# fanshiqing/mpiT

Measured on AMD Instinct MI355X. Metric: images/sec (whole node) ResNet-50 async-SGD at 1/2/4/8 MI355X, higher is better.
Workload: dtype fp32; 1 GPU; model=resnet50, global_batch=256, image_size=224, parallelism=async-ps-colocated-1srv-1wrk, optimizer=downpour, su=1, per_gpu_batch=256, master_weights=fp32, defer_ps_wait=False

## Files before the change

csrc/bindings.cpp:

```cpp
#include <pybind11/pybind11.h>
#include <pybind11/stl.h>

#include "core/engine.h"
#include "core/ps.h"
#include "core/window.h"
#include "kernels/kernels.h"
#include "kernels/stem_pack.h"

namespace py = pybind11;
using namespace mpit;

namespace {
hipStream_t S(uintptr_t s) { return reinterpret_cast<hipStream_t>(s); }
py::tuple st_tuple(const Status& s) { return py::make_tuple(s.source, s.tag, s.error, s.count, s.cancelled); }
}

static void apply_sfold(BnRed& r, const py::object& f) {
  if (f.is_none()) return;
  auto t = f.cast<py::tuple>();
  if (t.size() != 11 && t.size() != 12) throw std::invalid_argument("bn fold: 11 or 12 fields");
  r.scoef = t[0].cast<uintptr_t>();
  r.sgamma = t[1].cast<uintptr_t>();
  r.sbeta = t[2].cast<uintptr_t>();
  r.srmean = t[3].cast<uintptr_t>();
// ... 176 lines not shown
      py::arg("oepoch") = 0);
  m.def("gemm_nt_fold_lvl_floats", &gemm_nt_fold_lvl_floats);
  m.def("bound_floats", [] { return kBoundFloats; });
  m.def("gemm_tn_supported", &gemm_tn_supported);
  m.def("gemm_tn_ws_floats", &gemm_tn_ws_floats);
  m.def("device_cu_count", &device_cu_count);
  m.def("stream_create_cu_masked", &stream_create_cu_masked);
  m.def(
      "gemm_tn",
      [](int dev, uintptr_t s, int64_t M, int N, int K, uintptr_t Y, int64_t ldy, uintptr_t X, int64_t ldx,
         uintptr_t out, uintptr_t ws, float beta, bool f32, uintptr_t amax_y, uintptr_t amax_x, int64_t yps,
         int64_t xps) {
        gemm_tn(dev, S(s), M, N, K, Y, ldy, X, ldx, out, ws, beta, f32, amax_y, amax_x, yps, xps);
      },
      py::arg("dev"), py::arg("stream"), py::arg("M"), py::arg("N"), py::arg("K"), py::arg("Y"), py::arg("ldy"),
      py::arg("X"), py::arg("ldx"), py::arg("out"), py::arg("ws"), py::arg("beta"), py::arg("f32") = false,
      py::arg("amax_y") = 0, py::arg("amax_x") = 0, py::arg("yps") = 0, py::arg("xps") = 0);
  m.def(
      "cast_transpose",
      [](int dev, uintptr_t s, uintptr_t w, int R, int Cc, uintptr_t wb, uintptr_t wt, int taps, bool f32) {
        cast_transpose(dev, S(s), w, R, Cc, wb, wt, taps, f32);
      },
      py::arg("dev"), py::arg("stream"), py::arg("w"), py::arg("R"), py::arg("Cc"), py::arg("wb"), py::arg("wt"),
      py::arg("taps") = 1, py::arg("f32") = false);
  m.def("cast_job_bytes", &cast_job_bytes);
  m.def("cast_jobs_build", [](uintptr_t table, std::vector<std::array<int64_t, 11>> specs) {
    return cast_jobs_build(table, specs);
  });
  m.def(
      "cast_jobs_run",
      [](int dev, uintptr_t s, uintptr_t table, int njobs, int64_t nblocks, uintptr_t amax) {
        cast_jobs_run(dev, S(s), table, njobs, nblocks, amax);
      },
      py::arg("dev"), py::arg("s"), py::arg("table"), py::arg("njobs"), py::arg("nblocks"), py::arg("amax") = 0);
  m.def(
      "maxpool_fwd",
      [](int dev, uintptr_t s, int N, int H, int W, int C, int K, int stride, int pad, uintptr_t x, uintptr_t y,
         uintptr_t idx, bool f32, uintptr_t ibound, uintptr_t obound) {
        maxpool_fwd(dev, S(s), N, H, W, C, K, stride, pad, x, y, idx, f32, ibound, obound);
      },
      py::arg("dev"), py::arg("stream"), py::arg("N"), py::arg("H"), py::arg("W"), py::arg("C"), py::arg("K"),
      py::arg("stride"), py::arg("pad"), py::arg("x"), py::arg("y"), py::arg("idx"), py::arg("f32") = false,
      py::arg("ibound") = 0, py::arg("obound") = 0);
  m.def(
      "maxpool_bwd",
      [](int dev, uintptr_t s, int N, int H, int W, int C, int K, int stride, int pad, uintptr_t dy, uintptr_t idx,
         uintptr_t dx, bool f32, uintptr_t ypool, uintptr_t db, uintptr_t ws) {
        maxpool_bwd(dev, S(s), N, H, W, C, K, stride, pad, dy, idx, dx, f32, ypool, db, ws);
      },
      py::arg("dev"), py::arg("stream"), py::arg("N"), py::arg("H"), py::arg("W"), py::arg("C"), py::arg("K"),
      py::arg("stride"), py::arg("pad"), py::arg("dy"), py::arg("idx"), py::arg("dx"), py::arg("f32") = false,
      py::arg("ypool") = 0, py::arg("db") = 0, py::arg("ws") = 0);
  m.def("maxpool_bwd_ws_floats", &maxpool_bwd_ws_floats);
  m.def(
      "avgpool_bwd",
      [](int dev, uintptr_t s, int N, int HW, int C, uintptr_t dy, uintptr_t dx, bool f32) {
        avgpool_bwd(dev, S(s), N, HW, C, dy, dx, f32);
      },
      py::arg("dev"), py::arg("stream"), py::arg("N"), py::arg("HW"), py::arg("C"), py::arg("dy"), py::arg("dx"),
      py::arg("f32") = false);
  m.def("col_sums_ws_floats", &col_sums_ws_floats);
  m.def(
      "col_sums",
      [](int dev, uintptr_t s, uintptr_t part, int64_t nb, int64_t ld, int C, uintptr_t out, uintptr_t mid) {
        col_sums(dev, S(s), part, nb, ld, C, out, mid);
      },
      py::arg("dev"), py::arg("stream"), py::arg("part"), py::arg("nb"), py::arg("ld"), py::arg("C"), py::arg("out"),
      py::arg("mid") = 0);
  m.def("conv_supported", &conv_supported);
  m.def(
      "conv_fwd",
      [](int dev, uintptr_t s, int Nb, int H, int W, int C, int Co, int R, int S_, int stride, int pad, uintptr_t x,
         uintptr_t w, uintptr_t y, uintptr_t stats, uintptr_t cin, uintptr_t bias, bool relu, uintptr_t red_part,
         uintptr_t red_x, uintptr_t red_mask, uintptr_t red_mean, int64_t red_row0, uintptr_t red_part2,
         uintptr_t red_x2, uintptr_t red_mean2, bool f32, uintptr_t fold_coef, uintptr_t fold_gamma,
         uintptr_t fold_rstd, uintptr_t fold_dgamma, uintptr_t fold_dbeta, uintptr_t fold_lvl, int64_t bps,
         uintptr_t amax_a, uintptr_t amax_b, uintptr_t fold_zero, py::object bn_fold, bool red_relu,
         bool fold_tag, int64_t aps, uintptr_t omax, uint32_t oepoch) {
        BnRed r{red_part, red_x, red_mask, red_mean, red_row0, red_part2, red_x2, red_mean2};
        r.fcoef = fold_coef; r.fgamma = fold_gamma; r.frstd = fold_rstd;
        r.fdgamma = fold_dgamma; r.fdbeta = fold_dbeta; r.flvl = fold_lvl; r.fzero = fold_zero;
        r.amax_a = amax_a; r.amax_b = amax_b; r.aps = aps; r.omax = omax; r.oepoch = oepoch;
        r.relu_y = red_relu ? 1 : 0;
        r.ftag = fold_tag ? 1 : 0;
        apply_sfold(r, bn_fold);
        conv_fwd(dev, S(s), Nb, H, W, C, Co, R, S_, stride, pad, x, w, y, stats, cin, bias, relu, &r, f32, bps);
      },
      py::arg("dev"), py::arg("stream"), py::arg("Nb"), py::arg("H"), py::arg("W"), py::arg("C"), py::arg("Co"),
      py::arg("R"), py::arg("S"), py::arg("stride"), py::arg("pad"), py::arg("x"), py::arg("w"), py::arg("y"),
      py::arg("stats") = 0, py::arg("cin") = 0, py::arg("bias") = 0, py::arg("relu") = false, py::arg("red_part") = 0,
      py::arg("red_x") = 0, py::arg("red_mask") = 0, py::arg("red_mean") = 0, py::arg("red_row0") = 0,
      py::arg("red_part2") = 0, py::arg("red_x2") = 0, py::arg("red_mean2") = 0, py::arg("f32") = false,
      py::arg("fold_coef") = 0, py::arg("fold_gamma") = 0, py::arg("fold_rstd") = 0, py::arg("fold_dgamma") = 0,
      py::arg("fold_dbeta") = 0, py::arg("fold_lvl") = 0, py::arg("bps") = 0, py::arg("amax_a") = 0,
      py::arg("amax_b") = 0, py::arg("fold_zero") = 0, py::arg("bn_fold") = py::none(), py::arg("red_relu") = false,
      py::arg("fold_tag") = false, py::arg("aps") = 0, py::arg("omax") = 0, py::arg("oepoch") = 0);
  m.def("conv_dgrad_strided_wfloats", &conv_dgrad_strided_wfloats);
  m.def(
      "conv_dgrad_strided_weights",
      [](int dev, uintptr_t s, uintptr_t w, int Co, int C, int R, int S_, int stride, int pad, uintptr_t wb,
         uintptr_t wcls, bool f32) { conv_dgrad_strided_weights(dev, S(s), w, Co, C, R, S_, stride, pad, wb, wcls, f32); },
      py::arg("dev"), py::arg("stream"), py::arg("w"), py::arg("Co"), py::arg("C"), py::arg("R"), py::arg("S"),
      py::arg("stride"), py::arg("pad"), py::arg("wb"), py::arg("wcls"), py::arg("f32") = false);
  m.def("conv_dgrad_strided_tiles", &conv_dgrad_strided_tiles);
  m.def(
      "conv_dgrad_strided",
// ... 358 lines not shown
```

csrc/kernels/bn_act.hip:

```cpp
#include <hip/hip_runtime.h>

#include <atomic>
#include <cmath>
#include <stdexcept>
#include <cstdlib>
#include <string>
#include <type_traits>

#include "ew.h"
#include "kernels.h"
#include "planes.h"

namespace mpit {
namespace {

constexpr int kMaxStatBlocks = 512;
constexpr int kFinCh = 64;
constexpr int kFinK = 16;

template <typename T>
struct Vec;
template <>
struct Vec<uint16_t> {
  static constexpr int N = 8;
// ... 934 lines not shown
  check_shape(M, C, V, reinterpret_cast<uintptr_t>(x));
  if (relu && !mask) throw std::invalid_argument("bn_act backward: ReLU needs the forward mask");
  const int G = C / V;
  const int blk = block_for(G);
  const int R = blk / G;
  int64_t rpb;
  const int nb = stat_blocks(M, R, &rpb);
  const float* coef = coef_in ? coef_in : ws;
  float* part = ws + 3 * C;
  const size_t shm = size_t(R) * 2 * C * sizeof(float);
  if (coef_in) {
  } else if (gpart) {
    FinArgs fa{};
    fa.gamma = gamma;
    fa.mean = mean;
    fa.rstd = rstd;
    fa.dgamma = dgamma;
    fa.dbeta = dbeta;
    fa.coef = ws;
    fa.zero = reinterpret_cast<float*>(amax);
    launch_tiles_finalize<T, false>(s, gpart, npart, C, M, x, part, fa);
  } else {
    if (relu)
      hipLaunchKernelGGL((bn_bwd_reduce_kernel<T, true>), dim3(nb), dim3(blk), shm, s, dy, mask, x, mean, M, C, rpb,
                         part);
    else
      hipLaunchKernelGGL((bn_bwd_reduce_kernel<T, false>), dim3(nb), dim3(blk), shm, s, dy, mask, x, mean, M, C, rpb,
                         part);
    hipLaunchKernelGGL(bn_finalize_bwd_kernel, dim3((C + kFinCh - 1) / kFinCh), dim3(kFinCh * kFinK), 0, s, part, nb,
                       C, M, gamma, mean, rstd, dgamma, dbeta, ws);
    if (amax) hip_check(hipMemsetAsync(reinterpret_cast<void*>(amax), 0, kBoundFloats * sizeof(float), s), "amax zero");
  }
  const int64_t nvec = M * G;
  const int u = apply_u(sizeof(T) == 4);
  const dim3 g(apply_grid_u(nvec, blk, u)), b(blk);
  if (!dx) {
    hip_check(hipGetLastError(), "bn_act backward launch");
    return;
  }
  with_mode<sizeof(T) == 4>(split_ok(sizeof(T) == 4, C, blk), u, [&](auto sp, auto uu) {
    constexpr bool SP = decltype(sp)::value;
    constexpr int U = decltype(uu)::value;
    if (relu) {
      if (dres) hipLaunchKernelGGL((bn_bwd_apply_kernel<T, true, true, SP, U>), g, b, 0, s, dy, mask, x, coef, dx, dres, nvec, C, am);
      else hipLaunchKernelGGL((bn_bwd_apply_kernel<T, true, false, SP, U>), g, b, 0, s, dy, mask, x, coef, dx, dres, nvec, C, am);
    } else {
      if (dres) hipLaunchKernelGGL((bn_bwd_apply_kernel<T, false, true, SP, U>), g, b, 0, s, dy, mask, x, coef, dx, dres, nvec, C, am);
      else hipLaunchKernelGGL((bn_bwd_apply_kernel<T, false, false, SP, U>), g, b, 0, s, dy, mask, x, coef, dx, dres, nvec, C, am);
    }
  });
  hip_check(hipGetLastError(), "bn_act backward launch");
}

}

int64_t bn_workspace_floats(int C) { return int64_t(3) * C + int64_t(2) * kMaxStatBlocks * C; }

int64_t bn_mask_bytes(bool bf16, int64_t M, int C) { (void)bf16; return M * (C / 8); }

void bn_act_fwd(int dev, hipStream_t s, bool bf16, uintptr_t x, uintptr_t res, uintptr_t y, int64_t M, int C,
                uintptr_t gamma, uintptr_t beta, uintptr_t rmean, uintptr_t rvar, uintptr_t save_mean,
                uintptr_t save_rstd, uintptr_t ws, float momentum, float eps, bool relu, uintptr_t mask,
                uintptr_t stats, int64_t nstat, uintptr_t amax, uintptr_t coef, const PlaneSpec* planes) {
  hip_check(hipSetDevice(dev), "hipSetDevice");
  if (planes && (bf16 || (planes->obound && !y) || (planes->rplanes && !(res && planes->rbound)) ||
                 (planes->obound && res && !planes->rbound)))
    throw std::invalid_argument("bn_act forward: fp16 planes are for fp32 passes with the bounds of their inputs");
  auto F = [](uintptr_t p) { return reinterpret_cast<float*>(p); };
  auto* mk = reinterpret_cast<uint8_t*>(mask);
  if (coef) {
    if (!y) throw std::invalid_argument("bn_act forward: given coefficients need y");
    if (bf16) {
      check_shape(M, C, 8, x);
      launch_apply<uint16_t>(s, reinterpret_cast<const uint16_t*>(x), reinterpret_cast<const uint16_t*>(res),
                             reinterpret_cast<uint16_t*>(y), M, C, F(coef), relu, mk, AmaxOut{F(amax)});
    } else {
      check_shape(M, C, 8, x);
      launch_apply<float>(s, reinterpret_cast<const float*>(x), reinterpret_cast<const float*>(res),
                          reinterpret_cast<float*>(y), M, C, F(coef), relu, mk, amax_out(amax, planes));
    }
    hip_check(hipGetLastError(), "bn_act forward launch");
    return;
  }
  if (bf16)
    fwd_impl<uint16_t>(dev, s, reinterpret_cast<const uint16_t*>(x), reinterpret_cast<const uint16_t*>(res),
                       reinterpret_cast<uint16_t*>(y), M, C, F(gamma), F(beta), F(rmean), F(rvar), F(save_mean),
                       F(save_rstd), F(ws), momentum, eps, relu, mk, F(stats), nstat, amax, nullptr);
  else
    fwd_impl<float>(dev, s, reinterpret_cast<const float*>(x), reinterpret_cast<const float*>(res),
                    reinterpret_cast<float*>(y), M, C, F(gamma), F(beta), F(rmean), F(rvar), F(save_mean), F(save_rstd),
                    F(ws), momentum, eps, relu, mk, F(stats), nstat, amax, planes);
}

void bn_act_apply(int dev, hipStream_t s, bool bf16, uintptr_t x, uintptr_t res, uintptr_t y, int64_t M, int C,
                  uintptr_t coef, bool relu) {
  hip_check(hipSetDevice(dev), "hipSetDevice");
  if (bf16) {
    check_shape(M, C, 8, x);
    launch_apply<uint16_t>(s, reinterpret_cast<const uint16_t*>(x), reinterpret_cast<const uint16_t*>(res),
                           reinterpret_cast<uint16_t*>(y), M, C, reinterpret_cast<const float*>(coef), relu, nullptr);
  } else {
    check_shape(M, C, 8, x);
    launch_apply<float>(s, reinterpret_cast<const float*>(x), reinterpret_cast<const float*>(res),
                        reinterpret_cast<float*>(y), M, C, reinterpret_cast<const float*>(coef), relu, nullptr);
  }
  hip_check(hipGetLastError(), "bn_act apply launch");
// ... 81 lines not shown
```

csrc/kernels/kernels.h:

```cpp
#pragma once
#include <hip/hip_runtime.h>
#include <cstdint>
#include <array>
#include <vector>

namespace mpit {

enum Rule : int {
  kApply = 0,
  kApplySum = 1,
  kRMSProp = 2,
  kAdam = 3,
  kAdamax = 4,
  kAdagrad = 5,
  kAdadelta = 6,
  kNesterovPre = 7,
  kNesterovPost = 8,
  kDownpour = 9,
  kElastic = 10,
  kRegClip = 11,
  kScale = 12,
  kCopy = 13,
  kFill = 14,
  kAxpby = 15,
// ... 108 lines not shown
                        uintptr_t dy, uintptr_t wcls, uintptr_t dx, const BnRed* red = nullptr, bool f32 = false,
                        int64_t bps = 0);
void softmax_xent(int dev, hipStream_t s, int64_t rows, int C, uintptr_t x, int64_t ldx, bool bf16, uintptr_t tgt,
                  float scale, uintptr_t loss, uintptr_t d);

void seq_hidden_windows(int dev, hipStream_t s, uintptr_t tok, int64_t B, int T, uintptr_t E, int D, uintptr_t Wh,
                        uintptr_t bh, int H, int k, uintptr_t out, int Kp);
void seq_max_norm(int dev, hipStream_t s, uintptr_t c, int64_t ldc, uintptr_t tok, int64_t B, int T, int k,
                  int64_t pad_idx, uintptr_t bias, int F, float eps, uintptr_t out);
void gesd_gather(int dev, hipStream_t s, uintptr_t q, uintptr_t cand, uintptr_t idx, int64_t n, int w, int D,
                 uintptr_t out);

void seq_max_norm_arg(int dev, hipStream_t s, uintptr_t c, int64_t ldc, uintptr_t tok, int64_t B, int T, int k,
                      int64_t pad_idx, uintptr_t bias, int F, float eps, uintptr_t out, uintptr_t arg, uintptr_t den);
void gesd_pair_bwd(int dev, hipStream_t s, uintptr_t y, int64_t n, int F, float margin, uintptr_t err, uintptr_t sc,
                   uintptr_t gy);
void seq_norm_max_bwd(int dev, hipStream_t s, uintptr_t gy, uintptr_t y, uintptr_t arg, uintptr_t den, int64_t S, int T,
                      int F, int Fp, float eps, uintptr_t dm, uintptr_t dc);
void seq_conv_wgrad_pe(int dev, hipStream_t s, uintptr_t dm, uintptr_t arg, uintptr_t win, int64_t n, int T, int F,
                       int H, int k, int Kp, uintptr_t g, int64_t ldg, int64_t offW, int64_t offB);
void seq_hidden_bwd(int dev, hipStream_t s, uintptr_t dwin, int64_t ldw, uintptr_t win, int Kp, int64_t S, int T, int H,
                    int k, uintptr_t Wh, int D, uintptr_t da, uintptr_t de);
void seq_hidden_embed_grad_pe(int dev, hipStream_t s, uintptr_t da, uintptr_t de, uintptr_t tok, uintptr_t E,
                              int64_t V, int64_t n, int T, int H, int D, int64_t pad_idx, uintptr_t g, int64_t ldg,
                              int64_t offE, int64_t offWh, int64_t offBh);
int64_t relu_bias_bwd_ws_floats(int C);
int64_t col_sums_ws_floats(int C);
void col_sums(hipStream_t s, const float* part, int64_t nb, int64_t ld, int C, float* out, float* mid);
void col_sums(int dev, hipStream_t s, uintptr_t part, int64_t nb, int64_t ld, int C, uintptr_t out, uintptr_t mid);
void relu_bias_bwd(int dev, hipStream_t s, int64_t M, int C, uintptr_t dy, uintptr_t y, uintptr_t dz, uintptr_t db,
                   uintptr_t ws, bool f32 = false);
int64_t conv_wgrad_ws_floats(int dev, int Nb, int H, int W, int C, int Co, int R, int S, int stride, int pad);
void conv_wgrad(int dev, hipStream_t s, int Nb, int H, int W, int C, int Co, int R, int S, int stride, int pad,
                uintptr_t dy, uintptr_t x, uintptr_t dw, uintptr_t ws, float beta, bool f32 = false,
                uintptr_t amax_y = 0, uintptr_t amax_x = 0, int64_t yps = 0,
                int64_t xps = 0);

void conv_stem_fwd(int dev, hipStream_t s, int Nb, int Hp, int Wp, int Co, int Ho, int Wo, int stride, uintptr_t x,
                   uintptr_t w, uintptr_t y, uintptr_t stats, bool f32 = false, int64_t bps = 0, uintptr_t amax_a = 0,
                   uintptr_t amax_b = 0, const BnRed* fold = nullptr, int rows = 8, uintptr_t bias = 0,
                   bool relu = false);
int64_t conv_stem_wgrad_ws_floats(int dev, int Nb, int Ho, int Wo, int Co, int rows = 8);
void conv_stem_wgrad(int dev, hipStream_t s, int Nb, int Hp, int Wp, int Co, int Ho, int Wo, int stride, uintptr_t dy,
                     uintptr_t x, uintptr_t dw, uintptr_t ws, bool f32 = false, uintptr_t amax_y = 0,
                     uintptr_t amax_x = 0, int rows = 8);
int stem_wgrad_rows(int rows);

void maxpool_fwd(int dev, hipStream_t s, int N, int H, int W, int C, int K, int stride, int pad, uintptr_t x,
                 uintptr_t y, uintptr_t idx, bool f32 = false, uintptr_t ibound = 0, uintptr_t obound = 0);
void maxpool_bwd(int dev, hipStream_t s, int N, int H, int W, int C, int K, int stride, int pad, uintptr_t dy,
                 uintptr_t idx, uintptr_t dx, bool f32 = false, uintptr_t ypool = 0, uintptr_t db = 0,
                 uintptr_t ws = 0);
int64_t maxpool_bwd_ws_floats(int C);
void avgpool_bwd(int dev, hipStream_t s, int N, int HW, int C, uintptr_t dy, uintptr_t dx, bool f32 = false);

enum PeerOp : int { kPrSum = 0, kPrProd, kPrMax, kPrMin, kPrLand, kPrLor, kPrLxor, kPrBand, kPrBor, kPrBxor, kPrOps };
enum PeerDtype : int { kPrF32 = 0, kPrBf16, kPrF16, kPrF64, kPrI32, kPrI64, kPrU8, kPrDtypes };
constexpr int kPeerMax = 8;
bool peer_reduce_supported(int op, int dtype);
int peer_dtype_size(int dtype);
void peer_reduce(int dev, hipStream_t s, int op, int dtype, const std::vector<uintptr_t>& srcs,
                 const std::vector<uintptr_t>& dsts, int64_t n);

void type_copy(int dev, hipStream_t s, int dir, uintptr_t strided, uintptr_t packed,
               const std::vector<std::array<int64_t, 2>>& loops, uintptr_t table, int64_t R, int64_t L, int64_t per,
               int unit, int max_blocks = 0, bool wide = false);

}
```

mpit_amd/models/resnet.py:

```python
from __future__ import annotations

from typing import List, Type, Union

import os

import torch
import torch.nn as nn

from ..ops.bn import BatchNormAct2d, bn_pair
from ..ops.conv import Conv1x1, ConvNHWC, GradSlot, StemConv, feeds_bn, park_grad
from ..ops.linear import LinearAct
from ..ops.pool import GlobalAvgPoolNHWC, MaxPool2dNHWC

FUSED_BN = True


def _bn(c, act):
    return BatchNormAct2d(c, act=act) if FUSED_BN else nn.BatchNorm2d(c)


def _feeds_bn(*pairs):
    for p in pairs:
        if p is None:
            continue
        if isinstance(p, nn.Sequential):
            if not (len(p) == 2 and isinstance(p[1], BatchNormAct2d)):
                continue
            p = (p[0], p[1])
        c, bn = p
        if FUSED_BN and hasattr(c, "emit_stats") and isinstance(bn, BatchNormAct2d):
            feeds_bn(c, bn)


MFMA_CONV = os.environ.get("MPIT_MFMA_CONV", "1") != "0"
MFMA_CONV3 = MFMA_CONV and os.environ.get("MPIT_MFMA_CONV3", "1") != "0"
_FC_FP32 = os.environ.get("MPIT_FC_FP32", "0") != "0"


def conv3x3(i, o, stride=1):
    if MFMA_CONV3:
        return ConvNHWC(i, o, 3, stride=stride, padding=1)
    return nn.Conv2d(i, o, 3, stride=stride, padding=1, bias=False)


def conv1x1(i, o, stride=1):
    if MFMA_CONV:
        return Conv1x1(i, o) if stride == 1 else ConvNHWC(i, o, 1, stride=stride)
    return nn.Conv2d(i, o, 1, stride=stride, bias=False)


class BasicBlock(nn.Module):
    expansion = 1

    def __init__(self, inp, planes, stride=1, downsample=None):
        super().__init__()
        self.conv1 = conv3x3(inp, planes, stride)
        self.bn1 = _bn(planes, True)
        self.relu = nn.ReLU(inplace=True)
        self.conv2 = conv3x3(planes, planes)
        self.bn2 = _bn(planes, True)
        self.downsample = downsample
        _feeds_bn((self.conv1, self.bn1), (self.conv2, self.bn2), downsample)
# ... 64 lines not shown
        self.relu = nn.ReLU(inplace=True)
        self.maxpool = MaxPool2dNHWC(3, stride=2, padding=1) if MFMA_CONV else nn.MaxPool2d(3, stride=2, padding=1)
        self.layer1 = self._make(block, 64, layers[0])
        self.layer2 = self._make(block, 128, layers[1], 2)
        self.layer3 = self._make(block, 256, layers[2], 2)
        self.layer4 = self._make(block, 512, layers[3], 2)
        self.avgpool = GlobalAvgPoolNHWC() if MFMA_CONV else nn.AdaptiveAvgPool2d(1)
        self.fc = (LinearAct(512 * block.expansion, num_classes, act=False, pad_out=True) if MFMA_CONV
                   else nn.Linear(512 * block.expansion, num_classes))
        for m in self.modules():
            if isinstance(m, nn.Conv2d):
                nn.init.kaiming_normal_(m.weight, mode="fan_out", nonlinearity="relu")
            elif isinstance(m, nn.BatchNorm2d):
                nn.init.ones_(m.weight)
                nn.init.zeros_(m.bias)
        if zero_init_residual:
            for m in self.modules():
                if isinstance(m, Bottleneck):
                    nn.init.zeros_(m.bn3.weight)
                elif isinstance(m, BasicBlock):
                    nn.init.zeros_(m.bn2.weight)
        self._plan_planes()

    def _plan_planes(self):
        if not isinstance(self.bn1, BatchNormAct2d) or not isinstance(self.maxpool, MaxPool2dNHWC):
            return
        self.maxpool.out_planes = True
        blocks = [b for layer in (self.layer1, self.layer2, self.layer3, self.layer4) for b in layer]
        for b in blocks:
            bns = [b.bn1, b.bn2] + ([b.bn3] if isinstance(b, Bottleneck) else [])
            if b.downsample is not None and len(b.downsample) == 2:
                bns.append(b.downsample[1])
            for bn in bns:
                if isinstance(bn, BatchNormAct2d):
                    bn.out_planes = bn.grad_planes = True
        last = blocks[-1]
        feed_last, out_last = (last.bn2, last.bn3) if isinstance(last, Bottleneck) else (last.bn1, last.bn2)
        feed_last.out_planes = False
        out_last.out_planes = out_last.grad_planes = False

    def _make(self, block, planes, blocks, stride=1):
        down = None
        if stride != 1 or self.inplanes != planes * block.expansion:
            down = nn.Sequential(conv1x1(self.inplanes, planes * block.expansion, stride),
                                 _bn(planes * block.expansion, False))
        layers = [block(self.inplanes, planes, stride, down)]
        self.inplanes = planes * block.expansion
        for _ in range(1, blocks):
            layers.append(block(self.inplanes, planes))
        return nn.Sequential(*layers)

    def forward(self, x):
        if isinstance(self.bn1, BatchNormAct2d):
            x = self.maxpool(self.bn1(self.conv1(x)))
        else:
            x = self.maxpool(self.relu(self.bn1(self.conv1(x))))
        x = self.layer4(self.layer3(self.layer2(self.layer1(x))))
        x = torch.flatten(self.avgpool(x), 1)
        if _FC_FP32 and x.is_cuda and torch.is_autocast_enabled("cuda"):
            with torch.autocast("cuda", enabled=False):
                return self.fc(x.float())
        return self.fc(x)


def resnet18(num_classes=1000):
    return ResNet(BasicBlock, [2, 2, 2, 2], num_classes)


def resnet34(num_classes=1000):
    return ResNet(BasicBlock, [3, 4, 6, 3], num_classes)


def resnet50(num_classes=1000):
    return ResNet(Bottleneck, [3, 4, 6, 3], num_classes)


def resnet101(num_classes=1000):
    return ResNet(Bottleneck, [3, 4, 23, 3], num_classes)


def resnet152(num_classes=1000):
    return ResNet(Bottleneck, [3, 8, 36, 3], num_classes)
```

Measured before the change: 5856 images/sec.

## Fuse stem batchnorm, ReLU and maxpool into single forward and backward kernels

Adds HIP kernels that apply the folded BN affine and ReLU while computing the 3x3 stride-2 maxpool, storing only pooled outputs and uint8 argmax indices. The backward gathers pool gradients by recomputing the window from the index, masks them with the ReLU, and reduces the BN statistics in the same pass. This removes writing and rereading the full-resolution BN output and the separate pool and BN backward passes. In exchange it adds more complex index arithmetic and recomputation, and a new autograd path that is on by default for fp32.

```diff
diff --git a/csrc/bindings.cpp b/csrc/bindings.cpp
--- a/csrc/bindings.cpp
+++ b/csrc/bindings.cpp
@@ -252,6 +252,36 @@
       py::arg("stride"), py::arg("pad"), py::arg("dy"), py::arg("idx"), py::arg("dx"), py::arg("f32") = false,
       py::arg("ypool") = 0, py::arg("db") = 0, py::arg("ws") = 0);
   m.def("maxpool_bwd_ws_floats", &maxpool_bwd_ws_floats);
+  m.def("bn_pool_covered", &bn_pool_covered, py::arg("H"), py::arg("W"), py::arg("K"), py::arg("stride"),
+        py::arg("pad"));
+  m.def(
+      "bn_pool_fwd",
+      [](int dev, uintptr_t s, bool bf16, int N, int H, int W, int C, int K, int stride, int pad, uintptr_t x,
+         uintptr_t coef, uintptr_t y, uintptr_t idx, uintptr_t amax) {
+        bn_pool_fwd(dev, S(s), bf16, N, H, W, C, K, stride, pad, x, coef, y, idx, amax);
+      },
+      py::arg("dev"), py::arg("stream"), py::arg("bf16"), py::arg("N"), py::arg("H"), py::arg("W"), py::arg("C"),
+      py::arg("K"), py::arg("stride"), py::arg("pad"), py::arg("x"), py::arg("coef"), py::arg("y"), py::arg("idx"),
+      py::arg("amax") = 0);
+  m.def(
+      "pool_planes",
+      [](int dev, uintptr_t s, uintptr_t x, uintptr_t y, int64_t nel, uintptr_t ibound, uintptr_t obound) {
+        pool_planes(dev, S(s), x, y, nel, ibound, obound);
+      },
+      py::arg("dev"), py::arg("stream"), py::arg("x"), py::arg("y"), py::arg("nel"), py::arg("ibound"),
+      py::arg("obound"));
+  m.def(
+      "bn_pool_bwd",
+      [](int dev, uintptr_t s, bool bf16, int N, int H, int W, int C, int K, int stride, int pad, uintptr_t g,
+         uintptr_t idx, uintptr_t x, uintptr_t fcoef, uintptr_t gamma, uintptr_t mean, uintptr_t rstd, uintptr_t dx,
+         uintptr_t dgamma, uintptr_t dbeta, uintptr_t ws, uintptr_t amax) {
+        bn_pool_bwd(dev, S(s), bf16, N, H, W, C, K, stride, pad, g, idx, x, fcoef, gamma, mean, rstd, dx, dgamma, dbeta,
+                    ws, amax);
+      },
+      py::arg("dev"), py::arg("stream"), py::arg("bf16"), py::arg("N"), py::arg("H"), py::arg("W"), py::arg("C"),
+      py::arg("K"), py::arg("stride"), py::arg("pad"), py::arg("g"), py::arg("idx"), py::arg("x"), py::arg("fcoef"),
+      py::arg("gamma"), py::arg("mean"), py::arg("rstd"), py::arg("dx"), py::arg("dgamma"), py::arg("dbeta"),
+      py::arg("ws"), py::arg("amax") = 0);
   m.def(
       "avgpool_bwd",
       [](int dev, uintptr_t s, int N, int HW, int C, uintptr_t dy, uintptr_t dx, bool f32) {
diff --git a/csrc/kernels/bn_act.hip b/csrc/kernels/bn_act.hip
--- a/csrc/kernels/bn_act.hip
+++ b/csrc/kernels/bn_act.hip
@@ -1010,6 +1010,490 @@
   hip_check(hipGetLastError(), "bn_act backward launch");
 }
 
+struct FastDiv {
+  uint32_t d, mul, shr;
+};
+FastDiv fast_div(int d) {
+  FastDiv f{uint32_t(d), 0u, 0u};
+  if (d > 1) {
+    int l = 0;
+    while ((int64_t(1) << l) < d) ++l;
+    const int p = 31 + l;
+    f.mul = uint32_t(((uint64_t(1) << p) + uint32_t(d) - 1) / uint32_t(d));
+    f.shr = uint32_t(p - 32);
+  }
+  return f;
+}
+__device__ __forceinline__ uint32_t fdiv(uint32_t n, const FastDiv& f) {
+  return f.d == 1 ? n : __umulhi(n, f.mul) >> f.shr;
+}
+
+struct PoolGeo {
+  int N, H, W, C, Ho, Wo, K, stride, pad;
+  FastDiv dG, dC, dH, dW, dHo, dWo, dS;
+};
+
+template <bool NARROW>
+using pidx_t = std::conditional_t<NARROW, uint32_t, int64_t>;
+
+template <bool NARROW>
+__device__ __forceinline__ pidx_t<NARROW> fdivq(pidx_t<NARROW> a, const FastDiv& f) {
+  if constexpr (NARROW) return fdiv(a, f);
+  else return a / int64_t(f.d);
+}
+template <bool NARROW>
+__device__ __forceinline__ void divmod(pidx_t<NARROW> a, const FastDiv& f, pidx_t<NARROW>& q, int& m) {
+  if constexpr (NARROW) q = fdiv(a, f);
+  else q = a / int64_t(f.d);
+  m = int(a - q * f.d);
+}
+
+template <typename T, bool NARROW>
+__global__ __launch_bounds__(256) void bn_pool_fwd_kernel(const T* __restrict__ x, const float* __restrict__ coef,
+                                                          T* __restrict__ y, uint8_t* __restrict__ idx, PoolGeo g,
+                                                          int64_t total, AmaxOut am) {
+  using I = pidx_t<NARROW>;
+  const I t = I(blockIdx.x) * blockDim.x + threadIdx.x;
+  float mx = 0.f;
+  if (t < I(total)) {
+    I pix, r, n;
+    int c8, wo, ho;
+    divmod<NARROW>(t, g.dG, pix, c8);
+    divmod<NARROW>(pix, g.dWo, r, wo);
+    divmod<NARROW>(r, g.dHo, n, ho);
+    float sc[8], sh[8];
+    Vec<float>::load(coef + c8 * 8, sc);
+    Vec<float>::load(coef + g.C + c8 * 8, sh);
+    float best[8];
+    uint8_t arg[8];
+#pragma unroll
+    for (int e = 0; e < 8; ++e) {
+      best[e] = -__builtin_inff();
+      arg[e] = 0;
+    }
+    const int h0 = ho * g.stride - g.pad, w0 = wo * g.stride - g.pad;
+    for (int i = 0; i < g.K; ++i) {
+      const int h = h0 + i;
+      if (unsigned(h) >= unsigned(g.H)) continue;
+      for (int j = 0; j < g.K; ++j) {
+        const int w = w0 + j;
+        if (unsigned(w) >= unsigned(g.W)) continue;
+        float fv[8];
+        Vec<T>::load(x + (((n * g.H + h) * g.W + w) * g.C + c8 * 8), fv);
+        const uint8_t k = uint8_t(i * g.K + j);
+#pragma unroll
+        for (int e = 0; e < 8; ++e) {
+          float f = fmaxf(fmaf(fv[e], sc[e], sh[e]), 0.f);
+          mx = fmaxf(mx, fabsf(f));
+          if constexpr (sizeof(T) == 2) f = bf2f(f2bf(f));
+          if (f > best[e] || (f != f && best[e] == best[e])) {
+            best[e] = f;
+            arg[e] = k;
+          }
+        }
+      }
+    }
+    Vec<T>::store(y + (pix * g.C + c8 * 8), best);
+    uint2 a;
+    a.x = uint32_t(arg[0]) | (uint32_t(arg[1]) << 8) | (uint32_t(arg[2]) << 16) | (uint32_t(arg[3]) << 24);
+    a.y = uint32_t(arg[4]) | (uint32_t(arg[5]) << 8) | (uint32_t(arg[6]) << 16) | (uint32_t(arg[7]) << 24);
+    *reinterpret_cast<uint2*>(idx + (pix * g.C + c8 * 8)) = a;
+  }
+  if (am.amax) amax_finish(mx, am);
+}
+
+__global__ __launch_bounds__(256) void pool_planes_kernel(const float* __restrict__ x, float* __restrict__ y,
+                                                          int64_t nvec, const float* __restrict__ ibound,
+                                                          float* obound) {
+  const PlaneScale ps = plane_scale(slots_max_wave(ibound), obound);
+  const int64_t nel = nvec * 8;
+  uint16_t* yh = reinterpret_cast<uint16_t*>(y);
+  for (int64_t i = int64_t(blockIdx.x) * blockDim.x + threadIdx.x; i < nvec; i += int64_t(gridDim.x) * blockDim.x) {
+    float v[8];
+    Vec<float>::load(x + i * 8, v);
+    uint32_t hw[4], lw[4];
+#pragma unroll
+    for (int p = 0; p < 4; ++p) split_pair(v[2 * p], v[2 * p + 1], ps, hw[p], lw[p]);
+    *reinterpret_cast<uint4*>(yh + i * 8) = make_uint4(hw[0], hw[1], hw[2], hw[3]);
+    *reinterpret_cast<uint4*>(yh + nel + i * 8) = make_uint4(lw[0], lw[1], lw[2], lw[3]);
+  }
+}
+
+template <int CH>
+__device__ __forceinline__ void ld_arg(const uint8_t* __restrict__ p, uint32_t (&w)[CH / 4]) {
+  if constexpr (CH == 8) {
+    const uint2 a = *reinterpret_cast<const uint2*>(p);
+    w[0] = a.x;
+    w[1] = a.y;
+  } else {
+    w[0] = *reinterpret_cast<const uint32_t*>(p);
+  }
+}
+template <typename T, int CH>
+__device__ __forceinline__ void ld_ch(const T* __restrict__ p, float (&v)[CH]) {
+  if constexpr (CH == 8) {
+    Vec<T>::load(p, v);
+  } else {
+    static_assert(sizeof(T) == 4, "4-channel pieces are fp32");
+    const float4 r = *reinterpret_cast<const float4*>(p);
+    v[0] = r.x; v[1] = r.y; v[2] = r.z; v[3] = r.w;
+  }
+}
+
+template <int NW, bool NARROW>
+struct PoolWin {
+  pidx_t<NARROW> o[NW * NW];
+  int k[NW * NW];
+};
+template <int NW, bool NARROW>
+__device__ __forceinline__ void pool_win(const PoolGeo& g, pidx_t<NARROW> n, int h, int w, PoolWin<NW, NARROW>& win) {
+  const int ah = h + g.pad - g.K + g.stride, aw = w + g.pad - g.K + g.stride;
+  const int hlo = ah > 0 ? int(fdiv(uint32_t(ah), g.dS)) : 0, hhi = min(g.Ho - 1, int(fdiv(uint32_t(h + g.pad), g.dS)));
+  const int wlo = aw > 0 ? int(fdiv(uint32_t(aw), g.dS)) : 0, whi = min(g.Wo - 1, int(fdiv(uint32_t(w + g.pad), g.dS)));
+#pragma unroll
+  for (int p = 0; p < NW; ++p) {
+    const int ho = hlo + p, i = h - (ho * g.stride - g.pad);
+    const bool okh = ho <= hhi && i >= 0 && i < g.K;
+#pragma unroll
+    for (int q = 0; q < NW; ++q) {
+      const int wo = wlo + q, j = w - (wo * g.stride - g.pad);
+      const bool ok = okh && wo <= whi && j >= 0 && j < g.K;
+      win.o[p * NW + q] = ((n * g.Ho + min(ho, g.Ho - 1)) * g.Wo + min(wo, g.Wo - 1)) * g.C;
+      win.k[p * NW + q] = ok ? i * g.K + j : -1;
+    }
+  }
+}
+template <typename T, int NW, bool NARROW, int CH>
+__device__ __forceinline__ void pool_take(const T* __restrict__ gy, const uint8_t* __restrict__ idx,
+                                          const PoolWin<NW, NARROW>& win, int c0, float (&acc)[CH]) {
+  uint32_t a[NW * NW][CH / 4];
+  float gv[NW * NW][CH];
+#pragma unroll
+  for (int c = 0; c < NW * NW; ++c) {
+    ld_arg<CH>(idx + (win.o[c] + c0), a[c]);
+    ld_ch<T, CH>(gy + (win.o[c] + c0), gv[c]);
+  }
+#pragma unroll
+  for (int e = 0; e < CH; ++e) acc[e] = 0.f;
+#pragma unroll
+  for (int c = 0; c < NW * NW; ++c)
+#pragma unroll
+    for (int e = 0; e < CH; ++e) {
+      const int ae = int((a[c][e >> 2] >> (8 * (e & 3))) & 0xff);
+      if (ae == win.k[c]) acc[e] += gv[c][e];
+    }
+  if constexpr (sizeof(T) == 2) {
+#pragma unroll
+    for (int e = 0; e < CH; ++e) acc[e] = bf2f(f2bf(acc[e]));
+  }
+}
+
+template <typename T, int NW, bool NARROW, int CH>
+__device__ __forceinline__ void pool_gather(const T* __restrict__ gy, const uint8_t* __restrict__ idx,
+                                            const PoolGeo& g, pidx_t<NARROW> n, int h, int w, int c0,
+                                            float (&acc)[CH]) {
+  using I = pidx_t<NARROW>;
+  if constexpr (NW > 0) {
+    PoolWin<NW, NARROW> win;
+    pool_win<NW, NARROW>(g, n, h, w, win);
+    pool_take<T, NW, NARROW, CH>(gy, idx, win, c0, acc);
+  } else {
+#pragma unroll
+    for (int e = 0; e < CH; ++e) acc[e] = 0.f;
+    const int ah = h + g.pad - g.K + g.stride, aw = w + g.pad - g.K + g.stride;
+    const int hlo = ah > 0 ? int(fdiv(uint32_t(ah), g.dS)) : 0, hhi = min(g.Ho - 1, int(fdiv(uint32_t(h + g.pad), g.dS)));
+    const int wlo = aw > 0 ? int(fdiv(uint32_t(aw), g.dS)) : 0, whi = min(g.Wo - 1, int(fdiv(uint32_t(w + g.pad), g.dS)));
+    for (int ho = hlo; ho <= hhi; ++ho) {
+      const int i = h - (ho * g.stride - g.pad);
+      if (i < 0 || i >= g.K) continue;
+      for (int wo = wlo; wo <= whi; ++wo) {
+        const int j = w - (wo * g.stride - g.pad);
+        if (j < 0 || j >= g.K) continue;
+        const I o = ((n * g.Ho + ho) * g.Wo + wo) * g.C + c0;
+        uint32_t a[CH / 4];
+        float gv[CH];
+        ld_arg<CH>(idx + o, a);
+        ld_ch<T, CH>(gy + o, gv);
+        const int k = i * g.K + j;
+#pragma unroll
+        for (int e = 0; e < CH; ++e) {
+          const int ae = int((a[e >> 2] >> (8 * (e & 3))) & 0xff);
+          if (ae == k) acc[e] += gv[e];
+        }
+      }
+    }
+    if constexpr (sizeof(T) == 2) {
+#pragma unroll
+      for (int e = 0; e < CH; ++e) acc[e] = bf2f(f2bf(acc[e]));
+    }
+  }
+}
+
+template <typename T, int NW, bool NARROW, int CH>
+__device__ __forceinline__ void pool_dz(const T* __restrict__ gy, const uint8_t* __restrict__ idx, const PoolGeo& g,
+                                        pidx_t<NARROW> r, int c0, const float (&xx)[CH], const float (&sc)[CH],
+                                        const float (&sh)[CH], float (&dz)[CH]) {
+  pidx_t<NARROW> q, n;
+  int h, w;
+  divmod<NARROW>(r, g.dW, q, w);
+  divmod<NARROW>(q, g.dH, n, h);
+  pool_gather<T, NW, NARROW, CH>(gy, idx, g, n, h, w, c0, dz);
+#pragma unroll
+  for (int v = 0; v < CH; ++v) dz[v] = fmaf(xx[v], sc[v], sh[v]) > 0.f ? dz[v] : 0.f;
+}
+
+template <typename T, int NW, int MAXT, bool NARROW>
+__global__ __launch_bounds__(MAXT, 2) void bn_pool_bwd_reduce_kernel(const T* __restrict__ gy,
+                                                                  const uint8_t* __restrict__ idx,
+                                                                  const T* __restrict__ x,
+                                                                  const float* __restrict__ fcoef,
+                                                                  const float* __restrict__ mean, PoolGeo geo,
+                                                                  int64_t M, int64_t rows_per_block,
+                                                                  float* __restrict__ part) {
+  using I = pidx_t<NARROW>;
+  constexpr int V = Vec<T>::N;
+  extern __shared__ float lds[];
+  const int C = geo.C;
+  const int G = C / V;
+  const int g = threadIdx.x % G, rs = threadIdx.x / G, R = blockDim.x / G;
+  float mu[V], s1[V], s2[V], sc[V], sh[V];
+#pragma unroll
+  for (int v = 0; v < V; ++v) {
+    mu[v] = mean[g * V + v];
+    sc[v] = fcoef[g * V + v];
+    sh[v] = fcoef[C + g * V + v];
+    s1[v] = s2[v] = 0.f;
+  }
+  const int64_t r0 = int64_t(blockIdx.x) * rows_per_block;
+  const int64_t r1 = min(M, r0 + rows_per_block);
+  int64_t r = r0 + rs;
+  auto rows = [&](auto nu) {
+    constexpr int U = decltype(nu)::value;
+    float d[U][V], xx[U][V];
+#pragma unroll
+    for (int u = 0; u < U; ++u) {
+      const I ru = I(r + u * R);
+      Vec<T>::load(x + (ru * C + g * V), xx[u]);
+      pool_dz<T, NW, NARROW, V>(gy, idx, geo, ru, g * V, xx[u], sc, sh, d[u]);
+    }
+#pragma unroll
+    for (int u = 0; u < U; ++u)
+#pragma unroll
+      for (int v = 0; v < V; ++v) {
+        const float dz = d[u][v];
+        s1[v] += dz;
+        s2[v] = fmaf(dz, xx[u][v] - mu[v], s2[v]);
+      }
+  };
+  constexpr int UB = sizeof(T) == 4 ? 3 : 4;
+  if constexpr (MAXT <= 256)
+    for (; r + (UB - 1) * R < r1; r += UB * R) rows(std::integral_constant<int, UB>{});
+  for (; r + R < r1; r += 2 * R) rows(std::integral_constant<int, 2>{});
+  for (; r < r1; r += R) rows(std::integral_constant<int, 1>{});
+#pragma unroll
+  for (int v = 0; v < V; ++v) {
+    lds[(rs * 2 + 0) * C + g * V + v] = s1[v];
+    lds[(rs * 2 + 1) * C + g * V + v] = s2[v];
+  }
+  __syncthreads();
+  for (int c = threadIdx.x; c < C; c += blockDim.x) {
+    float a = 0.f, b = 0.f;
+    for (int k = 0; k < R; ++k) {
+      a += lds[(k * 2 + 0) * C + c];
+      b += lds[(k * 2 + 1) * C + c];
+    }
+    part[(size_t(blockIdx.x) * 2 + 0) * C + c] = a;
+    part[(size_t(blockIdx.x) * 2 + 1) * C + c] = b;
+  }
+}
+
+template <typename T, int NW, bool NARROW, int NP>
+__global__ __launch_bounds__(256) void bn_pool_bwd_apply_kernel(const T* __restrict__ gy,
+                                                                const uint8_t* __restrict__ idx,
+                                                                const T* __restrict__ x,
+                                                                const float* __restrict__ fcoef,
+                                                                const float* __restrict__ coef, T* __restrict__ dx,
+                                                                PoolGeo geo, FastDiv dL, int64_t nthr, AmaxOut am) {
+  using I = pidx_t<NARROW>;
+  constexpr int CH = sizeof(T) == 4 ? 4 : 8;
+  const int C = geo.C;
+  const I t0 = I(blockIdx.x) * blockDim.x + threadIdx.x;
+  const I stride = I(gridDim.x) * blockDim.x;
+  float mx = 0.f;
+  I r0;
+  int j;
+  divmod<NARROW>(t0, dL, r0, j);
+  float A[NP][CH], Cc[NP][CH], B[NP][CH], sc[NP][CH], sh[NP][CH];
+#pragma unroll
+  for (int p = 0; p < NP; ++p) {
+    const int c0 = (p * int(dL.d) + j) * CH;
+    ld_ch<float, CH>(fcoef + c0, sc[p]);
+    ld_ch<float, CH>(fcoef + C + c0, sh[p]);
+    ld_ch<float, CH>(coef + c0, A[p]);
+    ld_ch<float, CH>(coef + C + c0, Cc[p]);
+    ld_ch<float, CH>(coef + 2 * C + c0, B[p]);
+  }
+  for (I t = t0; t < I(nthr); t += stride) {
+    I q, n;
+    int h, w;
+    const I r = fdivq<NARROW>(t, dL);
+    divmod<NARROW>(r, geo.dW, q, w);
+    divmod<NARROW>(q, geo.dH, n, h);
+    [[maybe_unused]] PoolWin<(NW > 0 ? NW : 1), NARROW> win;
+    if constexpr (NW > 0) pool_win<NW, NARROW>(geo, n, h, w, win);
+    float xx[NP][CH], dz[NP][CH];
+#pragma unroll
+    for (int p = 0; p < NP; ++p) {
+      const int c0 = (p * int(dL.d) + j) * CH;
+      ld_ch<T, CH>(x + (r * C + c0), xx[p]);
+      if constexpr (NW > 0) pool_take<T, NW, NARROW, CH>(gy, idx, win, c0, dz[p]);
+      else pool_gather<T, NW, NARROW, CH>(gy, idx, geo, n, h, w, c0, dz[p]);
+    }
+#pragma unroll
+    for (int p = 0; p < NP; ++p) {
+      const int c0 = (p * int(dL.d) + j) * CH;
+#pragma unroll
+      for (int v = 0; v < CH; ++v) {
+        const float d = fmaf(xx[p][v], sc[p][v], sh[p][v]) > 0.f ? dz[p][v] : 0.f;
+        xx[p][v] = fmaf(A[p][v], d, fmaf(Cc[p][v], xx[p][v], B[p][v]));
+        mx = fmaxf(mx, fabsf(xx[p][v]));
+      }
+      if constexpr (CH == 8) Vec<T>::store(dx + (r * C + c0), xx[p]);
+      else *reinterpret_cast<float4*>(dx + (r * C + c0)) = make_float4(xx[p][0], xx[p][1], xx[p][2], xx[p][3]);
+    }
+  }
+  if (am.amax) amax_finish(mx, am);
+}
+
+PoolGeo bn_pool_geo(int N, int H, int W, int C, int K, int stride, int pad) {
+  if (N <= 0 || H <= 0 || W <= 0 || C <= 0 || C % 8 || K <= 0 || K > 15 || stride <= 0 || pad < 0 || 2 * pad > K)
+    throw std::invalid_argument("bn_pool: unsupported geometry (C % 8 == 0, K <= 15, pad <= K/2)");
+  if (!bn_pool_covered(H, W, K, stride, pad))
+    throw std::invalid_argument("bn_pool: the windows must cover every input pixel");
+  PoolGeo g{N, H, W, C, (H + 2 * pad - K) / stride + 1, (W + 2 * pad - K) / stride + 1, K, stride, pad};
+  g.dG = fast_div(C / 8);
+  g.dC = fast_div(C);
+  g.dH = fast_div(H);
+  g.dW = fast_div(W);
+  g.dHo = fast_div(g.Ho);
+  g.dWo = fast_div(g.Wo);
+  g.dS = fast_div(stride);
+  return g;
+}
+
+bool pool_narrow(const PoolGeo& g) { return int64_t(g.N) * g.H * g.W * g.C + 2048 < (int64_t(1) << 31); }
+
+template <typename T>
+void bn_pool_fwd_t(hipStream_t s, const PoolGeo& g, uintptr_t x, uintptr_t coef, uintptr_t y, uintptr_t idx,
+                   uintptr_t amax) {
+  const int64_t total = int64_t(g.N) * g.Ho * g.Wo * (g.C / 8);
+  const int64_t blocks = (total + 255) / 256;
+  if (blocks > INT32_MAX) throw std::invalid_argument("bn_pool_fwd: tensor too large");
+  auto* k = pool_narrow(g) ? bn_pool_fwd_kernel<T, true> : bn_pool_fwd_kernel<T, false>;
+  hipLaunchKernelGGL(k, dim3(unsigned(blocks)), dim3(256), 0, s, reinterpret_cast<const T*>(x),
+                     reinterpret_cast<const float*>(coef), reinterpret_cast<T*>(y), reinterpret_cast<uint8_t*>(idx), g,
+                     total, AmaxOut{reinterpret_cast<float*>(amax)});
+  hip_check(hipGetLastError(), "bn_pool_fwd launch");
+}
+
+template <typename T>
+void bn_pool_bwd_t(hipStream_t s, const PoolGeo& geo, const T* gy, const uint8_t* idx, const T* x, const float* fcoef,
+                   const float* gamma, const float* mean, const float* rstd, T* dx, float* dgamma, float* dbeta,
+                   float* ws, uintptr_t amax) {
+  constexpr int V = Vec<T>::N;
+  const int C = geo.C;
+  const int64_t M = int64_t(geo.N) * geo.H * geo.W;
+  check_shape(M, C, V, reinterpret_cast<uintptr_t>(x));
+  const int G = C / V;
+  const int blk = block_for(G);
+  const int R = blk / G;
+  int64_t rpb;
+  const int nb = stat_blocks(M, R, &rpb);
+  float* part = ws + 3 * C;
+  const size_t shm = size_t(R) * 2 * C * sizeof(float);
+  constexpr int CH = sizeof(T) == 4 ? 4 : 8;
+  const int np = C % (CH * 2) == 0 ? 2 : 1;
+  const int L = C / (CH * np);
+  const int64_t nthr = M * L;
+  constexpr int kApplyRounds = 4;
+  const int64_t blocks = 256 % L == 0 ? (nthr + 256 * kApplyRounds - 1) / (256 * kApplyRounds) : (nthr + 255) / 256;
+  if (blocks > INT32_MAX) throw std::invalid_argument("bn_pool_bwd: tensor too large");
+  const bool narrow = pool_narrow(geo);
+  const bool nw2 = (geo.K + geo.stride - 1) / geo.stride <= 2;
+  {
+    auto* k = nw2 && blk <= 256 ? (narrow ? bn_pool_bwd_reduce_kernel<T, 2, 256, true> : bn_pool_bwd_reduce_kernel<T, 2, 256, false>)
+                                : (narrow ? bn_pool_bwd_reduce_kernel<T, 0, 1024, true> : bn_pool_bwd_reduce_kernel<T, 0, 1024, false>);
+    hipLaunchKernelGGL(k, dim3(nb), dim3(blk), shm, s, gy, idx, x, fcoef, mean, geo, M, rpb, part);
+  }
+  hipLaunchKernelGGL(bn_finalize_bwd_kernel, dim3((C + kFinCh - 1) / kFinCh), dim3(kFinCh * kFinK), 0, s, part, nb, C,
+                     M, gamma, mean, rstd, dgamma, dbeta, ws);
+  if (amax) hip_check(hipMemsetAsync(reinterpret_cast<void*>(amax), 0, kBoundFloats * sizeof(float), s), "amax zero");
+  const AmaxOut am{reinterpret_cast<float*>(amax)};
+  auto apply = [&](auto nw, auto nr, auto npc) {
+    hipLaunchKernelGGL((bn_pool_bwd_apply_kernel<T, decltype(nw)::value, decltype(nr)::value, decltype(npc)::value>),
+                       dim3(unsigned(blocks)), dim3(256), 0, s, gy, idx, x, fcoef, static_cast<const float*>(ws), dx,
+                       geo, fast_div(L), nthr, am);
+  };
+  auto apply_np = [&](auto nw, auto nr) {
+    if (np == 2) apply(nw, nr, std::integral_constant<int, 2>{});
+    else apply(nw, nr, std::integral_constant<int, 1>{});
+  };
+  auto apply_nr = [&](auto nw) {
+    if (narrow) apply_np(nw, std::true_type{});
+    else apply_np(nw, std::false_type{});
+  };
+  if (nw2) apply_nr(std::integral_constant<int, 2>{});
+  else apply_nr(std::integral_constant<int, 0>{});
+  hip_check(hipGetLastError(), "bn_pool_bwd launch");
+}
+
+}
+
+bool bn_pool_covered(int H, int W, int K, int stride, int pad) {
+  if (H <= 0 || W <= 0 || K <= 0 || stride <= 0 || pad < 0) return false;
+  const int Ho = (H + 2 * pad - K) / stride + 1, Wo = (W + 2 * pad - K) / stride + 1;
+  if (H + 2 * pad < K || W + 2 * pad < K) return false;
+  return (Ho - 1) * stride - pad + K - 1 >= H - 1 && (Wo - 1) * stride - pad + K - 1 >= W - 1;
+}
+
+void bn_pool_fwd(int dev, hipStream_t s, bool bf16, int N, int H, int W, int C, int K, int stride, int pad,
+                 uintptr_t x, uintptr_t coef, uintptr_t y, uintptr_t idx, uintptr_t amax) {
+  const PoolGeo g = bn_pool_geo(N, H, W, C, K, stride, pad);
+  if (!x || !coef || !y || !idx || (x | y | coef) % 16 || idx % 8)
+    throw std::invalid_argument("bn_pool_fwd: missing or misaligned buffers");
+  hip_check(hipSetDevice(dev), "hipSetDevice");
+  if (bf16) bn_pool_fwd_t<uint16_t>(s, g, x, coef, y, idx, amax);
+  else bn_pool_fwd_t<float>(s, g, x, coef, y, idx, amax);
+}
+
+void pool_planes(int dev, hipStream_t s, uintptr_t x, uintptr_t y, int64_t nel, uintptr_t ibound, uintptr_t obound) {
+  if (nel <= 0 || nel % 8 || !x || !y || x == y || (x | y) % 16 || (nel * 2) % 16 || !ibound || !obound)
+    throw std::invalid_argument("pool_planes: needs nel % 8 == 0, two aligned buffers and both bounds");
+  hip_check(hipSetDevice(dev), "hipSetDevice");
+  const int64_t nvec = nel / 8;
+  const unsigned grid = unsigned(std::min<int64_t>((nvec + 255) / 256, 65536));
+  hipLaunchKernelGGL(pool_planes_kernel, dim3(grid), dim3(256), 0, s, reinterpret_cast<const float*>(x),
+                     reinterpret_cast<float*>(y), nvec, reinterpret_cast<const float*>(ibound),
+                     reinterpret_cast<float*>(obound));
+  hip_check(hipGetLastError(), "pool_planes launch");
+}
+
+void bn_pool_bwd(int dev, hipStream_t s, bool bf16, int N, int H, int W, int C, int K, int stride, int pad,
+                 uintptr_t g, uintptr_t idx, uintptr_t x, uintptr_t fcoef, uintptr_t gamma, uintptr_t mean,
+                 uintptr_t rstd, uintptr_t dx, uintptr_t dgamma, uintptr_t dbeta, uintptr_t ws, uintptr_t amax) {
+  const PoolGeo geo = bn_pool_geo(N, H, W, C, K, stride, pad);
+  if (!g || !idx || !x || !fcoef || !mean || !rstd || !dx || !ws || (g | x | dx | fcoef | ws) % 16 || idx % 8)
+    throw std::invalid_argument("bn_pool_bwd: missing or misaligned buffers");
+  hip_check(hipSetDevice(dev), "hipSetDevice");
+  auto F = [](uintptr_t p) { return reinterpret_cast<float*>(p); };
+  const auto* ix = reinterpret_cast<const uint8_t*>(idx);
+  if (bf16)
+    bn_pool_bwd_t<uint16_t>(s, geo, reinterpret_cast<const uint16_t*>(g), ix, reinterpret_cast<const uint16_t*>(x),
+                            F(fcoef), F(gamma), F(mean), F(rstd), reinterpret_cast<uint16_t*>(dx), F(dgamma),
+                            F(dbeta), F(ws), amax);
+  else
+    bn_pool_bwd_t<float>(s, geo, reinterpret_cast<const float*>(g), ix, reinterpret_cast<const float*>(x), F(fcoef),
+                         F(gamma), F(mean), F(rstd), reinterpret_cast<float*>(dx), F(dgamma), F(dbeta), F(ws), amax);
 }
 
 int64_t bn_workspace_floats(int C) { return int64_t(3) * C + int64_t(2) * kMaxStatBlocks * C; }
diff --git a/csrc/kernels/kernels.h b/csrc/kernels/kernels.h
--- a/csrc/kernels/kernels.h
+++ b/csrc/kernels/kernels.h
@@ -184,6 +184,14 @@
                  uintptr_t idx, uintptr_t dx, bool f32 = false, uintptr_t ypool = 0, uintptr_t db = 0,
                  uintptr_t ws = 0);
 int64_t maxpool_bwd_ws_floats(int C);
+
+bool bn_pool_covered(int H, int W, int K, int stride, int pad);
+void bn_pool_fwd(int dev, hipStream_t s, bool bf16, int N, int H, int W, int C, int K, int stride, int pad,
+                 uintptr_t x, uintptr_t coef, uintptr_t y, uintptr_t idx, uintptr_t amax = 0);
+void pool_planes(int dev, hipStream_t s, uintptr_t x, uintptr_t y, int64_t nel, uintptr_t ibound, uintptr_t obound);
+void bn_pool_bwd(int dev, hipStream_t s, bool bf16, int N, int H, int W, int C, int K, int stride, int pad,
+                 uintptr_t g, uintptr_t idx, uintptr_t x, uintptr_t fcoef, uintptr_t gamma, uintptr_t mean,
+                 uintptr_t rstd, uintptr_t dx, uintptr_t dgamma, uintptr_t dbeta, uintptr_t ws, uintptr_t amax = 0);
 void avgpool_bwd(int dev, hipStream_t s, int N, int HW, int C, uintptr_t dy, uintptr_t dx, bool f32 = false);
 
 enum PeerOp : int { kPrSum = 0, kPrProd, kPrMax, kPrMin, kPrLand, kPrLor, kPrLxor, kPrBand, kPrBor, kPrBxor, kPrOps };
diff --git a/mpit_amd/models/resnet.py b/mpit_amd/models/resnet.py
--- a/mpit_amd/models/resnet.py
+++ b/mpit_amd/models/resnet.py
@@ -8,6 +8,7 @@
 import torch.nn as nn
 
 from ..ops.bn import BatchNormAct2d, bn_pair
+from ..ops.bn_pool import bn_relu_pool
 from ..ops.conv import Conv1x1, ConvNHWC, GradSlot, StemConv, feeds_bn, park_grad
 from ..ops.linear import LinearAct
 from ..ops.pool import GlobalAvgPoolNHWC, MaxPool2dNHWC
@@ -178,7 +179,7 @@
 
     def forward(self, x):
         if isinstance(self.bn1, BatchNormAct2d):
-            x = self.maxpool(self.bn1(self.conv1(x)))
+            x = bn_relu_pool(self.bn1, self.maxpool, self.conv1(x))
         else:
             x = self.maxpool(self.relu(self.bn1(self.conv1(x))))
         x = self.layer4(self.layer3(self.layer2(self.layer1(x))))
diff --git a/mpit_amd/ops/bn_pool.py b/mpit_amd/ops/bn_pool.py
--- /dev/null
+++ b/mpit_amd/ops/bn_pool.py
@@ -0,0 +1,118 @@
+from __future__ import annotations
+
+import os
+
+import torch
+
+from .._ext import native
+from . import bn as _bn
+from . import conv as _conv
+from .bn import BatchNormAct2d, _amax_buf, _cl, _want_amax, tile_stats_of
+from .conv import ReluLink, set_amax, set_planes
+from .pool import MaxPool2dNHWC, _int
+
+_STEM_FUSE = {"0": False, "1": True, "all": True}.get(os.environ.get("MPIT_STEM_FUSE", "fp32"), "fp32")
+
+COUNTERS = {"fwd": 0, "bwd": 0}
+
+
+class _BNPoolFn(torch.autograd.Function):
+    @staticmethod
+    def forward(ctx, x, weight, bias, running_mean, running_var, momentum, eps, k, stride, pad, tstats=None,
+                amax=None, obound=None):
+        x = _cl(x)
+        n, c, h, w_ = x.shape
+        M = n * h * w_
+        m = native()
+        dev = x.device.index
+        stream = torch.cuda.current_stream(x.device).cuda_stream
+        bf16 = x.dtype == torch.bfloat16
+        f32 = dict(dtype=torch.float32, device=x.device)
+        w = weight.float().contiguous() if weight is not None else None
+        b = bias.float().contiguous() if bias is not None else None
+        ts = tstats if (tstats is not None and tstats[1] == m.gemm_nt_tiles(M)) else None
+        fold = ts[2] if ts is not None else None
+        if ts is not None:
+            _bn.COUNTERS["fwd_tile_stats"] += 1
+        if fold is not None:
+            _bn.COUNTERS["fwd_folded"] += 1
+            mean, rstd, coef = fold.mean, fold.rstd, fold.coef
+        else:
+            mean, rstd = torch.empty(c, **f32), torch.empty(c, **f32)
+            ws = torch.empty(m.bn_workspace_floats(c), **f32)
+            m.bn_act_fwd(dev, stream, bf16, x.data_ptr(), 0, 0, M, c, w.data_ptr() if w is not None else 0,
+                         b.data_ptr() if b is not None else 0,
+                         running_mean.data_ptr() if running_mean is not None else 0,
+                         running_var.data_ptr() if running_var is not None else 0, mean.data_ptr(), rstd.data_ptr(),
+                         ws.data_ptr(), float(momentum), float(eps), False, 0,
+                         stats=ts[0].data_ptr() if ts is not None else 0, nstat=ts[1] if ts is not None else 0,
+                         amax=amax.data_ptr() if amax is not None else 0)
+            coef = ws[: 2 * c]
+        ho, wo = (h + 2 * pad - k) // stride + 1, (w_ + 2 * pad - k) // stride + 1
+        y = torch.empty((n, c, ho, wo), dtype=x.dtype, device=x.device, memory_format=torch.channels_last)
+        idx = torch.empty((n, ho, wo, c), dtype=torch.uint8, device=x.device)
+        m.bn_pool_fwd(dev, stream, bf16, n, h, w_, c, k, stride, pad, x.data_ptr(), coef.data_ptr(), y.data_ptr(),
+                      idx.data_ptr(), amax=amax.data_ptr() if amax is not None else 0)
+        if obound is not None:
+            yp = torch.empty_like(y, memory_format=torch.channels_last)
+            m.pool_planes(dev, stream, y.data_ptr(), yp.data_ptr(), y.numel(), amax.data_ptr(), obound.data_ptr())
+            y = yp
+        ctx.save_for_backward(x, idx, coef, w, mean, rstd)
+        ctx.geo = (k, stride, pad)
+        ctx.has_w = weight is not None
+        ctx.has_b = bias is not None
+        COUNTERS["fwd"] += 1
+        return y
+
+    @staticmethod
+    def backward(ctx, dy):
+        x, idx, coef, w, mean, rstd = ctx.saved_tensors
+        k, stride, pad = ctx.geo
+        dy = _cl(dy).to(x.dtype)
+        n, c, h, w_ = x.shape
+        m = native()
+        f32 = dict(dtype=torch.float32, device=x.device)
+        dx = torch.empty_like(x, memory_format=torch.channels_last)
+        dgamma = torch.empty(c, **f32) if ctx.has_w else None
+        dbeta = torch.empty(c, **f32) if ctx.has_b else None
+        ws = torch.empty(m.bn_workspace_floats(c), **f32)
+        amax = _amax_buf(x)
+        m.bn_pool_bwd(x.device.index, torch.cuda.current_stream(x.device).cuda_stream, x.dtype == torch.bfloat16, n, h,
+                      w_, c, k, stride, pad, dy.data_ptr(), idx.data_ptr(), x.data_ptr(), coef.data_ptr(),
+                      w.data_ptr() if w is not None else 0, mean.data_ptr(), rstd.data_ptr(), dx.data_ptr(),
+                      dgamma.data_ptr() if dgamma is not None else 0, dbeta.data_ptr() if dbeta is not None else 0,
+                      ws.data_ptr(), amax=amax.data_ptr() if amax is not None else 0)
+        if amax is not None:
+            set_amax(dx, amax)
+        COUNTERS["bwd"] += 1
+        return dx, dgamma, dbeta, None, None, None, None, None, None, None, None, None, None
+
+
+def fusable(bn, pool, x: torch.Tensor) -> bool:
+    if not (_STEM_FUSE and isinstance(bn, BatchNormAct2d) and isinstance(pool, MaxPool2dNHWC)):
+        return False
+    if _STEM_FUSE == "fp32" and x.dtype != torch.float32:
+        return False
+    if not (bn.act and bn.fused(x) and pool.fused(x) and ReluLink.of(x) is None):
+        return False
+    k, s, p = _int(pool.kernel_size), _int(pool.stride), _int(pool.padding)
+    return bool(native().bn_pool_covered(x.shape[2], x.shape[3], k, s, p))
+
+
+def bn_relu_pool(bn, pool, x: torch.Tensor) -> torch.Tensor:
+    if not fusable(bn, pool, x):
+        return pool(bn(x))
+    momentum, rm, rv = bn._train_args()
+    ts = tile_stats_of(x)
+    fold = ts[2] if ts is not None else None
+    amax = fold.amax if (fold is not None and _want_amax(x)) else _amax_buf(x)
+    planes = (pool.out_planes and _conv._F32_PLANES and x.dtype == torch.float32 and amax is not None
+              and pool.training)
+    ob = torch.empty(_conv.BOUND_FLOATS, dtype=torch.float32, device=x.device) if planes else None
+    y = _BNPoolFn.apply(x, bn.weight, bn.bias, rm, rv, momentum, bn.eps, _int(pool.kernel_size), _int(pool.stride),
+                        _int(pool.padding), ts, amax, ob)
+    if ob is not None:
+        set_planes(y, ob)
+    elif amax is not None:
+        set_amax(y, amax)
+    return y
```

Result: faster. 5915 images/sec, median of 6 (+1.0%).
